# penghao-wu/vstar

Hardware: AMD Instinct MI355X
Metric: searched crops/sec (336x336 tiles, 7B VSM bf16) (higher is better)
Workload: dtype bf16; 1 GPU; BASELINE config 2: 32-crop batches/GPU, CLIP-ViT-L/14@336 (P=576) + LLaMA-7B prefill S=640 + OWL-ViT-B/16@768 + det/SAM heads, records all-gathered per step; seq_len=640, parallelism=dp1

## Files before the change

### include/vstar_hip.h

```cpp
#ifndef VSTAR_HIP_H
#define VSTAR_HIP_H

#include <stdint.h>
#include <stddef.h>

#ifdef __cplusplus
extern "C" {
#endif

#define VSTAR_ABI_VERSION 1

enum { VSTAR_F32 = 0, VSTAR_F16 = 1, VSTAR_BF16 = 2 };

enum {
  VSTAR_OK = 0,
  VSTAR_ERR_INVALID = -1,
  VSTAR_ERR_STATE = -2,
  VSTAR_ERR_MISSING = -3,
  VSTAR_ERR_HIP = -4,
  VSTAR_ERR_NOMEM = -5
};

typedef struct vstar_config {
  int32_t abi_version;
// ... 49 lines not shown
#define VSTAR_F_DEVICE_INPUTS  2u
#define VSTAR_F_DEVICE_OUTPUT  4u
#define VSTAR_F_NO_SYNC        8u
#define VSTAR_F_INTERNAL_PIXELS 16u
#define VSTAR_F_SHARE_PREFIX   32u
int vstar_vsm_score_batch(vstar_handle* h, int B, const uint16_t* clip_pix, const uint16_t* owl_pix,
                          const int32_t* ids, int L, const int32_t* loc_pos,
                          const int32_t* verify_pos, int n_verify, unsigned flags, vstar_result* out);

int vstar_vsm_score_grouped(vstar_handle* h, int G, int T, const uint16_t* clip_pix, const uint16_t* owl_pix,
                            const int32_t* prefix_ids, int Lp, const int32_t* suffix_ids, int Ls, const int32_t* loc_in_suffix,
                            const int32_t* verify_in_suffix, int n_verify, unsigned flags, vstar_result* out);

int vstar_image_set(vstar_handle* h, const uint8_t* rgb, int height, int width);
int vstar_preprocess_crops(vstar_handle* h, int B, const int32_t* boxes_xyxy);

#define VSTAR_MAX_IMAGE_SLOTS 64
int vstar_image_set_slot(vstar_handle* h, int slot, const uint8_t* rgb, int height, int width);
int vstar_preprocess_crops_slots(vstar_handle* h, int B, const int32_t* boxes_xyxy, const int32_t* slots);
int vstar_image_set_slot_async(vstar_handle* h, int slot, const uint8_t* rgb, int height, int width);

int vstar_vsm_generate(vstar_handle* h, const uint16_t* clip_pix_bf16, const int32_t* ids, int L, int max_new_tokens,
                       int eos_id, unsigned flags, int32_t* out_ids, int32_t* n_out);

int vstar_upsample_mask(vstar_handle* h, const float* lowres, int h_out, int w_out, float* out);
int vstar_upsample_mask_ex(vstar_handle* h, const float* lowres, int h_out, int w_out, int clamp_min0, float* out);

int vstar_heatmap_stats(vstar_handle* h, const float* lowres, int h_out, int w_out, int n_rects, const int32_t* rects_xywh,
                        double* out);
int vstar_heatmap_stats_batch(vstar_handle* h, int n, const float* lowres, const int32_t* out_hw, const int32_t* n_rects,
                              const int32_t* rects_xywh, double* out);

int64_t vstar_debug_read(vstar_handle* h, const char* name, float* out, int64_t cap);

void* vstar_stream(vstar_handle* h);

#define VSTAR_COMM_ID_BYTES 128
int vstar_comm_unique_id(uint8_t* id_out );
int vstar_comm_init(vstar_handle* h, const uint8_t* id, int world, int rank);
int vstar_allgather_results(vstar_handle* h, const vstar_result* local_dev, int n_local, vstar_result* gathered_dev, unsigned flags);
int vstar_comm_destroy(vstar_handle* h);

int vstar_profile_enable(vstar_handle* h, int on);
int vstar_profile_read(vstar_handle* h, double* gemm_ms, int64_t* gemm_launches, double* gemm_flops);
int vstar_profile_read_fp8(vstar_handle* h, double* gemm_ms, int64_t* gemm_launches, double* gemm_flops);

enum { VSTAR_EPI_NONE = 0, VSTAR_EPI_QUICK_GELU = 1, VSTAR_EPI_GELU = 2, VSTAR_EPI_RELU = 3, VSTAR_EPI_SILU_MUL = 4,
       VSTAR_EPI_NOSYNC = 0x100,
       VSTAR_EPI_TILE128 = 0x200,
       VSTAR_EPI_TILE256 = 0x400,
       VSTAR_EPI_TILE4W = 0x800    };

int vstar_op_gemm(void* stream, const uint16_t* dev_A, int64_t lda, const uint16_t* dev_W, const uint16_t* dev_bias,
                  const uint16_t* dev_residual, int64_t ldr, void* dev_C, int64_t ldc, int out_f32,
                  int M, int N, int K, int epilogue);
int vstar_op_gemm_norm(void* stream, const uint16_t* dev_A, int64_t lda, const uint16_t* dev_W, const uint16_t* dev_bias,
                       const uint16_t* dev_residual, int64_t ldr, void* dev_C, int64_t ldc, int M, int N, int K, int epilogue,
                       const float* dev_row_scale, float* dev_sumsq_out, int sumsq_ld);
int vstar_op_rms_rstd(void* stream, const uint16_t* dev_x, const float* dev_partials, int ld, int rows, int cols, float eps,
                      float* dev_r);
int vstar_op_ln_fold(void* stream, uint16_t* dev_W, uint16_t* dev_bias, const uint16_t* dev_g, const uint16_t* dev_b_ln,
                     int n_rows, int K);
int vstar_op_gemm_last_tile(void);
int vstar_op_gemm_plan(int M, int N, int K, int epilogue, int has_residual, int fused_rope, int cus);
int vstar_op_gemm_fp8(void* stream, const uint16_t* dev_A, const uint16_t* dev_W, const uint16_t* dev_bias,
                      const uint16_t* dev_residual, uint16_t* dev_C, int M, int N, int K, int epilogue, int iters, float* gemm_ms);
size_t vstar_op_mx_scale_bytes(int rows, int cols);
int64_t vstar_op_mx_scale_offset(int row, int k_block, int rows);
int vstar_op_quantize_mx(void* stream, const uint16_t* dev_X, uint8_t* dev_q, uint8_t* dev_scales, int rows, int cols);
int vstar_op_gemm_mx(void* stream, const uint8_t* dev_Aq, const uint8_t* dev_a_scales, const float* dev_row_scale, const uint16_t* dev_W,
                     const uint16_t* dev_residual, uint16_t* dev_C, uint8_t* dev_C8, uint8_t* dev_c_scales, float* dev_sumsq, int M, int N, int K,
                     int epilogue, int iters, float* gemm_ms);
int vstar_op_gemm_fp8_mxout(void* stream, const uint16_t* dev_A, const uint16_t* dev_W, uint8_t* dev_C8, uint8_t* dev_c_scales, int M, int N,
                            int K, int iters, float* gemm_ms);
int vstar_op_attention_mx(void* stream, const uint16_t* dev_qkv, uint8_t* dev_out8, uint8_t* dev_scales, int B, int S, int H);
int vstar_w8a8_mx_active(vstar_handle* h);
int vstar_op_layernorm(void* stream, const uint16_t* dev_x, const uint16_t* dev_gamma, const uint16_t* dev_beta,
                       uint16_t* dev_y, int rows, int cols, float eps);
int vstar_op_rmsnorm(void* stream, const uint16_t* dev_x, const uint16_t* dev_gamma, uint16_t* dev_y,
                     int rows, int cols, float eps);
int vstar_op_attention(void* stream, uint16_t* dev_qkv, uint16_t* dev_out, void* dev_workspace, size_t workspace_bytes,
                       int B, int S, int H, int D, int causal, float rope_theta);
size_t vstar_op_attention_workspace(int B, int S, int H, int D);

int vstar_op_owl_class_logits(void* stream, const float* dev_emb, int ld, int Q, const uint16_t* dev_query, float* dev_out,
                              int out_stride_crop, int B, int rows_per_crop, int img_div);
int vstar_op_owl_box_finish(void* stream, const float* dev_raw, int ld, float* dev_out, int out_stride_crop, int B, int grid, int img_div);
int vstar_op_upsample2x_im2col3x3(void* stream, const uint16_t* dev_src, uint16_t* dev_A, int B, int h, int w, int C);
int vstar_op_hyper_mask(void* stream, const uint16_t* dev_hyper, const uint16_t* dev_up, float* dev_out, int out_stride_crop, int B,
                        int npix, int C);
int vstar_op_im2col_patch(void* stream, const uint16_t* dev_pix, uint16_t* dev_A, int B, int I, int ps, int Kpad);
int vstar_op_vit_assemble_tokens(void* stream, const uint16_t* dev_patch, const uint16_t* dev_cls, const uint16_t* dev_pos,
                                 uint16_t* dev_tokens, int B, int P, int C);
int vstar_op_llm_embed_text(void* stream, const int32_t* dev_ids, int L, int img_col, int P, const uint16_t* dev_table, int vocab,
                            uint16_t* dev_x, int B, int C);
int vstar_op_add_bcast(void* stream, const uint16_t* dev_a, const uint16_t* dev_b, uint16_t* dev_out, int64_t rows, int cols,
                       int64_t b_rows);
int vstar_op_add_bcast_repeat(void* stream, const uint16_t* dev_a, const uint16_t* dev_b, uint16_t* dev_out, int n_out, int rep,
                              int rows_per, int cols);
int vstar_op_bcast_rows(void* stream, const uint16_t* dev_src, uint16_t* dev_dst, int nrep, int64_t rep_stride, int nrows, int cols,
                        int64_t ld);
int vstar_op_owl_cls_mul(void* stream, const uint16_t* dev_x, uint16_t* dev_y, int B, int N, int C);
int vstar_op_gather_rows(void* stream, const uint16_t* dev_x, const int32_t* dev_idx, uint16_t* dev_y, int rows, int cols);
int vstar_op_argmax_rows(void* stream, const float* dev_x, int rows, int cols, int ld, int32_t* dev_out, int out_stride);
int vstar_op_layernorm_ex(void* stream, const uint16_t* dev_x, const uint16_t* dev_gamma, const uint16_t* dev_beta, uint16_t* dev_y,
                          int rows, int cols, float eps, const int32_t* dev_row_index, int act);
int vstar_op_rmsnorm_ex(void* stream, const uint16_t* dev_x, const uint16_t* dev_gamma, uint16_t* dev_y, int rows, int cols, float eps,
                        const int32_t* dev_row_index);
int vstar_op_ln_rstd(void* stream, const uint16_t* dev_x, const float* dev_partials, int ld, int rows, int cols, float eps,
                     float* dev_r);
int vstar_op_scale_cols(void* stream, uint16_t* dev_W, const uint16_t* dev_w, int64_t rows, int K);
int vstar_op_fill(void* stream, uint16_t* dev_v, int64_t n, float value);
int vstar_op_quantize_rows_fp8(void* stream, const uint16_t* dev_x, int64_t ldx, uint8_t* dev_q, int64_t ldq, float* dev_scale, int rows,
                               int cols);
int vstar_op_rmsnorm_quant_fp8(void* stream, const uint16_t* dev_x, const uint16_t* dev_gamma, uint8_t* dev_q, float* dev_scale, int rows,
                               int cols, float eps);
int vstar_op_small_attention(void* stream, const uint16_t* dev_q, const uint16_t* dev_k, const uint16_t* dev_v, uint16_t* dev_out, int B,
                             int Nq, int Nk, int H, int D);

#ifdef __cplusplus
}
#endif
#endif
```

### vstar_amd/_lib.py

```python
from __future__ import annotations

import ctypes
import os
from ctypes import POINTER, c_char_p, c_double, c_float, c_int, c_int32, c_int64, c_size_t, c_uint, c_uint16, c_void_p

from .config import CVqaConfig, CVstarConfig, MASK_RES, MAX_VERIFY, N_BOXES

LIB_PATH = os.environ.get("VSTAR_LIB") or os.path.join(os.path.dirname(os.path.abspath(__file__)), "libvstar_hip.so")

EXPORTS = [
    "vstar_create", "vstar_destroy", "vstar_last_error", "vstar_load_tensor", "vstar_finalize_weights",
    "vstar_vsm_score_batch", "vstar_upsample_mask", "vstar_debug_read", "vstar_stream", "vstar_profile_enable",
    "vstar_profile_read", "vstar_profile_read_fp8", "vstar_op_gemm", "vstar_op_layernorm", "vstar_op_rmsnorm", "vstar_op_attention",
    "vstar_op_attention_workspace", "vstar_image_set", "vstar_preprocess_crops", "vstar_heatmap_stats", "vstar_heatmap_stats_batch", "vstar_vsm_generate", "vstar_op_gemm_fp8",
    "vstar_op_gemm_last_tile", "vstar_op_gemm_plan", "vstar_op_gemm_norm", "vstar_op_rms_rstd", "vstar_op_ln_fold", "vstar_upsample_mask_ex", "vstar_vsm_score_grouped",
    "vstar_image_set_slot", "vstar_image_set_slot_async", "vstar_preprocess_crops_slots", "vstar_comm_unique_id", "vstar_comm_init", "vstar_allgather_results",
    "vstar_comm_destroy", "vstar_build_source_hash", "vstar_op_mx_scale_bytes", "vstar_op_mx_scale_offset", "vstar_op_quantize_mx",
    "vstar_op_gemm_mx", "vstar_op_gemm_fp8_mxout", "vstar_op_attention_mx", "vstar_w8a8_mx_active",
    "vstar_op_owl_class_logits", "vstar_op_owl_box_finish", "vstar_op_upsample2x_im2col3x3", "vstar_op_hyper_mask",
    "vstar_op_im2col_patch", "vstar_op_vit_assemble_tokens", "vstar_op_llm_embed_text", "vstar_op_add_bcast",
    "vstar_op_add_bcast_repeat", "vstar_op_bcast_rows", "vstar_op_owl_cls_mul", "vstar_op_gather_rows", "vstar_op_argmax_rows",
    "vstar_op_layernorm_ex", "vstar_op_rmsnorm_ex", "vstar_op_ln_rstd", "vstar_op_scale_cols", "vstar_op_fill",
    "vstar_op_quantize_rows_fp8", "vstar_op_rmsnorm_quant_fp8", "vstar_op_small_attention",
]

EXPORTS_VQA = [
    "vstar_vqa_create", "vstar_vqa_destroy", "vstar_vqa_last_error", "vstar_vqa_load_tensor", "vstar_vqa_finalize_weights",
    "vstar_vqa_encode_images", "vstar_vqa_forward", "vstar_vqa_debug_read", "vstar_vqa_last_forward_ms", "vstar_vqa_op_gemm",
    "vstar_vqa_forward_sample", "vstar_vqa_op_sample", "vstar_vqa_forward_beam", "vstar_vqa_kv_reorder", "vstar_vqa_kv_copy",
    "vstar_vqa_op_beam_select", "vstar_vqa_forward_score", "vstar_vqa_op_score",
    "vstar_vqa_decode_weight_bits", "vstar_vqa_op_quantize_w8", "vstar_vqa_op_gemm_w8",
    "vstar_vqa_op_quantize_w4", "vstar_vqa_op_gemm_w4",
    "vstar_vqa_kv_cache_format", "vstar_vqa_kv_cache_bytes", "vstar_vqa_op_kv_quantize",
    "vstar_vqa_forward_verify", "vstar_vqa_op_verify",
    "vstar_vqa_forward_edits", "vstar_vqa_forward_sample_edits", "vstar_vqa_forward_verify_edits", "vstar_vqa_op_edit",
    "vstar_vqa_logit_edit_capacity",
]

F32, F16, BF16 = 0, 1, 2
MAX_IMAGE_SLOTS = 64
EPI_NONE, EPI_QUICK_GELU, EPI_GELU, EPI_RELU, EPI_SILU_MUL = range(5)
EPI_NOSYNC, EPI_TILE128, EPI_TILE256, EPI_TILE4W = 0x100, 0x200, 0x400, 0x800
TILE_4W = 2564
F_SKIP_OWL, F_DEVICE_INPUTS, F_DEVICE_OUTPUT, F_NO_SYNC, F_INTERNAL_PIXELS, F_SHARE_PREFIX = 1, 2, 4, 8, 16, 32


class VstarResult(ctypes.Structure):
    _fields_ = [
        ("pred_logits", c_float * N_BOXES),
        ("pred_boxes", c_float * (N_BOXES * 4)),
        ("lowres_mask", c_float * (MASK_RES * MASK_RES)),
        ("tf_argmax", c_int32 * MAX_VERIFY),
    ]


RESULT_FLOATS = ctypes.sizeof(VstarResult) // 4


class VqaSampling(ctypes.Structure):
    _fields_ = [
        ("temperature", c_float),
        ("top_k", c_int32),
        ("top_p", c_float),
        ("step", ctypes.c_uint32),
        ("seed", ctypes.c_uint64),
        ("stream", ctypes.c_uint64),
    ]


class VqaLogitEdits(ctypes.Structure):
    _fields_ = [
        ("off", c_void_p),
        ("tok", c_void_p),
        ("penalty", c_void_p),
    ]


class VstarError(RuntimeError):
    pass


_lib = None


def load() -> ctypes.CDLL:
    global _lib
    if _lib is not None:
        return _lib
    if not os.path.exists(LIB_PATH):
        raise VstarError(f"{LIB_PATH} not built — run __graft_entry__.build() (hipcc --offload-arch=gfx950); "
                         "there is no CPU fallback for the HIP engine")
    import torch
    lib = ctypes.CDLL(LIB_PATH)
    H = c_void_p
    lib.vstar_create.argtypes = [POINTER(CVstarConfig), c_int, POINTER(H)]
    lib.vstar_create.restype = c_int
    lib.vstar_destroy.argtypes = [H]
    lib.vstar_destroy.restype = None
    lib.vstar_last_error.argtypes = [H]
    lib.vstar_last_error.restype = c_char_p
    lib.vstar_build_source_hash.argtypes = []
# ... 6 lines not shown
                                          c_void_p]
    lib.vstar_vsm_score_batch.restype = c_int
    lib.vstar_vsm_score_grouped.argtypes = [H, c_int, c_int, c_void_p, c_void_p, c_void_p, c_int, c_void_p, c_int, c_void_p, c_void_p, c_int,
                                            c_uint, c_void_p]
    lib.vstar_vsm_score_grouped.restype = c_int
    lib.vstar_vsm_generate.argtypes = [H, c_void_p, c_void_p, c_int, c_int, c_int, c_uint, c_void_p, c_void_p]
    lib.vstar_vsm_generate.restype = c_int
    lib.vstar_image_set.argtypes = [H, c_void_p, c_int, c_int]
    lib.vstar_image_set.restype = c_int
    lib.vstar_preprocess_crops.argtypes = [H, c_int, c_void_p]
    lib.vstar_preprocess_crops.restype = c_int
    lib.vstar_image_set_slot.argtypes = [H, c_int, c_void_p, c_int, c_int]
    lib.vstar_image_set_slot.restype = c_int
    lib.vstar_image_set_slot_async.argtypes = [H, c_int, c_void_p, c_int, c_int]
    lib.vstar_image_set_slot_async.restype = c_int
    lib.vstar_preprocess_crops_slots.argtypes = [H, c_int, c_void_p, c_void_p]
    lib.vstar_preprocess_crops_slots.restype = c_int
    lib.vstar_comm_unique_id.argtypes = [c_void_p]
    lib.vstar_comm_unique_id.restype = c_int
    lib.vstar_comm_init.argtypes = [H, c_void_p, c_int, c_int]
    lib.vstar_comm_init.restype = c_int
    lib.vstar_allgather_results.argtypes = [H, c_void_p, c_int, c_void_p, ctypes.c_uint]
    lib.vstar_allgather_results.restype = c_int
    lib.vstar_comm_destroy.argtypes = [H]
    lib.vstar_comm_destroy.restype = c_int
    lib.vstar_heatmap_stats.argtypes = [H, c_void_p, c_int, c_int, c_int, c_void_p, c_void_p]
    lib.vstar_heatmap_stats.restype = c_int
    lib.vstar_heatmap_stats_batch.argtypes = [H, c_int, c_void_p, c_void_p, c_void_p, c_void_p, c_void_p]
    lib.vstar_heatmap_stats_batch.restype = c_int
    lib.vstar_upsample_mask.argtypes = [H, c_void_p, c_int, c_int, c_void_p]
    lib.vstar_upsample_mask.restype = c_int
    lib.vstar_upsample_mask_ex.argtypes = [H, c_void_p, c_int, c_int, c_int, c_void_p]
    lib.vstar_upsample_mask_ex.restype = c_int
    lib.vstar_debug_read.argtypes = [H, c_char_p, c_void_p, c_int64]
    lib.vstar_debug_read.restype = c_int64
    lib.vstar_stream.argtypes = [H]
    lib.vstar_stream.restype = c_void_p
    lib.vstar_profile_enable.argtypes = [H, c_int]
    lib.vstar_profile_enable.restype = c_int
    lib.vstar_profile_read.argtypes = [H, POINTER(c_double), POINTER(c_int64), POINTER(c_double)]
    lib.vstar_profile_read.restype = c_int
    lib.vstar_profile_read_fp8.argtypes = [H, POINTER(c_double), POINTER(c_int64), POINTER(c_double)]
    lib.vstar_profile_read_fp8.restype = c_int
    lib.vstar_op_gemm.argtypes = [c_void_p, c_void_p, c_int64, c_void_p, c_void_p, c_void_p, c_int64, c_void_p, c_int64,
                                  c_int, c_int, c_int, c_int, c_int]
    lib.vstar_op_gemm.restype = c_int
    lib.vstar_op_gemm_norm.argtypes = [c_void_p, c_void_p, c_int64, c_void_p, c_void_p, c_void_p, c_int64, c_void_p, c_int64, c_int, c_int, c_int,
                                       c_int, c_void_p, c_void_p, c_int]
    lib.vstar_op_gemm_norm.restype = c_int
    lib.vstar_op_rms_rstd.argtypes = [c_void_p, c_void_p, c_void_p, c_int, c_int, c_int, c_float, c_void_p]
    lib.vstar_op_rms_rstd.restype = c_int
    lib.vstar_op_ln_fold.argtypes = [c_void_p, c_void_p, c_void_p, c_void_p, c_void_p, c_int, c_int]
    lib.vstar_op_ln_fold.restype = c_int
    lib.vstar_op_gemm_last_tile.argtypes = []
    lib.vstar_op_gemm_last_tile.restype = c_int
    lib.vstar_op_gemm_plan.argtypes = [c_int] * 7
    lib.vstar_op_gemm_plan.restype = c_int
    lib.vstar_op_gemm_fp8.argtypes = [c_void_p, c_void_p, c_void_p, c_void_p, c_void_p, c_void_p, c_int, c_int, c_int, c_int, c_int,
                                      POINTER(c_float)]
    lib.vstar_op_gemm_fp8.restype = c_int
    lib.vstar_op_mx_scale_bytes.argtypes = [c_int, c_int]
    lib.vstar_op_mx_scale_bytes.restype = c_size_t
    lib.vstar_op_mx_scale_offset.argtypes = [c_int, c_int, c_int]
    lib.vstar_op_mx_scale_offset.restype = ctypes.c_int64
    lib.vstar_op_quantize_mx.argtypes = [c_void_p, c_void_p, c_void_p, c_void_p, c_int, c_int]
    lib.vstar_op_quantize_mx.restype = c_int
    lib.vstar_op_gemm_mx.argtypes = [c_void_p] * 10 + [c_int, c_int, c_int, c_int, c_int, POINTER(c_float)]
    lib.vstar_op_gemm_mx.restype = c_int
    lib.vstar_op_gemm_fp8_mxout.argtypes = [c_void_p, c_void_p, c_void_p, c_void_p, c_void_p, c_int, c_int, c_int, c_int, POINTER(c_float)]
    lib.vstar_op_gemm_fp8_mxout.restype = c_int
    lib.vstar_op_attention_mx.argtypes = [c_void_p, c_void_p, c_void_p, c_void_p, c_int, c_int, c_int]
    lib.vstar_op_attention_mx.restype = c_int
    lib.vstar_w8a8_mx_active.argtypes = [c_void_p]
    lib.vstar_w8a8_mx_active.restype = c_int
    lib.vstar_op_layernorm.argtypes = [c_void_p, c_void_p, c_void_p, c_void_p, c_void_p, c_int, c_int, c_float]
    lib.vstar_op_layernorm.restype = c_int
    lib.vstar_op_rmsnorm.argtypes = [c_void_p, c_void_p, c_void_p, c_void_p, c_int, c_int, c_float]
    lib.vstar_op_rmsnorm.restype = c_int
    lib.vstar_op_attention.argtypes = [c_void_p, c_void_p, c_void_p, c_void_p, c_size_t, c_int, c_int, c_int, c_int, c_int,
                                       c_float]
    lib.vstar_op_attention.restype = c_int
    lib.vstar_op_attention_workspace.argtypes = [c_int, c_int, c_int, c_int]
    lib.vstar_op_attention_workspace.restype = c_size_t
    V, I, L, F = c_void_p, c_int, c_int64, c_float
    for name, args in {
        "owl_class_logits": [V, I, I, V, V, I, I, I, I], "owl_box_finish": [V, I, V, I, I, I, I],
        "upsample2x_im2col3x3": [V, V, I, I, I, I], "hyper_mask": [V, V, V, I, I, I, I],
        "im2col_patch": [V, V, I, I, I, I], "vit_assemble_tokens": [V, V, V, V, I, I, I],
        "llm_embed_text": [V, I, I, I, V, I, V, I, I], "add_bcast": [V, V, V, L, I, L],
        "add_bcast_repeat": [V, V, V, I, I, I, I], "bcast_rows": [V, V, I, L, I, I, L], "owl_cls_mul": [V, V, I, I, I],
        "gather_rows": [V, V, V, I, I], "argmax_rows": [V, I, I, I, V, I],
        "layernorm_ex": [V, V, V, V, I, I, F, V, I], "rmsnorm_ex": [V, V, V, I, I, F, V], "ln_rstd": [V, V, I, I, I, F, V],
        "scale_cols": [V, V, L, I], "fill": [V, L, F], "quantize_rows_fp8": [V, L, V, L, V, I, I],
        "rmsnorm_quant_fp8": [V, V, V, V, I, I, F], "small_attention": [V, V, V, V, I, I, I, I, I],
    }.items():
        fn = getattr(lib, "vstar_op_" + name)
        fn.argtypes = [c_void_p] + args
        fn.restype = c_int
    lib.vstar_vqa_create.argtypes = [POINTER(CVqaConfig), c_int, POINTER(H)]
    lib.vstar_vqa_create.restype = c_int
    lib.vstar_vqa_destroy.argtypes = [H]
    lib.vstar_vqa_destroy.restype = None
    lib.vstar_vqa_last_error.argtypes = [H]
    lib.vstar_vqa_last_error.restype = c_char_p
    lib.vstar_vqa_load_tensor.argtypes = [H, c_char_p, c_void_p, c_int, c_int, POINTER(c_int64)]
    lib.vstar_vqa_load_tensor.restype = c_int
    lib.vstar_vqa_finalize_weights.argtypes = [H]
    lib.vstar_vqa_finalize_weights.restype = c_int
    lib.vstar_vqa_encode_images.argtypes = [H, c_int, c_void_p, c_int]
    lib.vstar_vqa_encode_images.restype = c_int
    lib.vstar_vqa_forward.argtypes = [H, c_int, c_void_p, c_void_p, c_void_p, c_void_p, c_void_p, c_int, c_void_p, c_void_p,
                                      c_void_p]
    lib.vstar_vqa_forward.restype = c_int
    lib.vstar_vqa_forward_sample.argtypes = [H, c_int, c_void_p, c_void_p, c_void_p, c_void_p, c_void_p, c_int, c_void_p,
                                             c_void_p, c_void_p]
    lib.vstar_vqa_forward_sample.restype = c_int
    lib.vstar_vqa_op_sample.argtypes = [c_void_p, c_int, c_int, c_int, c_int64, c_void_p, c_void_p, c_void_p, c_void_p]
    lib.vstar_vqa_op_sample.restype = c_int
    lib.vstar_vqa_forward_beam.argtypes = [H, c_int, c_void_p, c_void_p, c_void_p, c_void_p, c_void_p, c_int, c_void_p,
                                           c_void_p, c_int, c_void_p, c_int, c_void_p, c_void_p, c_void_p, c_void_p]
    lib.vstar_vqa_forward_beam.restype = c_int
    lib.vstar_vqa_kv_reorder.argtypes = [H, c_int, c_void_p, c_void_p, c_int, c_int]
    lib.vstar_vqa_kv_reorder.restype = c_int
    lib.vstar_vqa_kv_copy.argtypes = [H, c_int, c_int, c_int, c_int]
    lib.vstar_vqa_kv_copy.restype = c_int
    lib.vstar_vqa_op_beam_select.argtypes = [c_void_p, c_int, c_int, c_int, c_int64, c_void_p, c_int, c_void_p, c_int, c_void_p,
                                             c_void_p, c_void_p, c_void_p]
    lib.vstar_vqa_op_beam_select.restype = c_int
    lib.vstar_vqa_forward_score.argtypes = [H, c_int, c_void_p, c_void_p, c_void_p, c_void_p, c_void_p, c_int, c_void_p,
                                            c_void_p, c_void_p, c_void_p]
    lib.vstar_vqa_forward_score.restype = c_int
    lib.vstar_vqa_op_score.argtypes = [c_void_p, c_int, c_int, c_int, c_int64, c_void_p, c_void_p, c_void_p, c_void_p]
    lib.vstar_vqa_op_score.restype = c_int
    lib.vstar_vqa_forward_verify.argtypes = [H, c_int, c_void_p, c_void_p, c_void_p, c_void_p, c_void_p, c_int, c_void_p,
                                             c_void_p, c_void_p, c_int, c_void_p, c_void_p, c_void_p]
    lib.vstar_vqa_forward_verify.restype = c_int
    lib.vstar_vqa_op_verify.argtypes = [c_void_p, c_int, c_int, c_int, c_int64, c_void_p, c_int, c_void_p, c_void_p, c_void_p,
                                        c_void_p]
    lib.vstar_vqa_op_verify.restype = c_int
    lib.vstar_vqa_forward_edits.argtypes = lib.vstar_vqa_forward.argtypes + [c_void_p]
    lib.vstar_vqa_forward_edits.restype = c_int
    lib.vstar_vqa_forward_sample_edits.argtypes = lib.vstar_vqa_forward_sample.argtypes + [c_void_p]
    lib.vstar_vqa_forward_sample_edits.restype = c_int
    lib.vstar_vqa_forward_verify_edits.argtypes = lib.vstar_vqa_forward_verify.argtypes + [c_void_p]
    lib.vstar_vqa_forward_verify_edits.restype = c_int
    lib.vstar_vqa_op_edit.argtypes = [c_void_p, c_int, c_int, c_int, c_int64, c_void_p, c_void_p, c_void_p]
    lib.vstar_vqa_op_edit.restype = c_int
    lib.vstar_vqa_logit_edit_capacity.argtypes = [H]
    lib.vstar_vqa_logit_edit_capacity.restype = c_int64
    lib.vstar_vqa_op_gemm.argtypes = [c_void_p, c_void_p, c_void_p, c_void_p, c_void_p, c_int, c_int, c_int, c_int, c_int,
                                      c_void_p, c_float]
    lib.vstar_vqa_op_gemm.restype = c_int
    lib.vstar_vqa_decode_weight_bits.argtypes = [H]
    lib.vstar_vqa_decode_weight_bits.restype = c_int
    lib.vstar_vqa_op_quantize_w8.argtypes = [c_void_p, c_int, c_int, c_void_p, c_void_p, c_void_p]
    lib.vstar_vqa_op_quantize_w8.restype = c_int
    lib.vstar_vqa_op_gemm_w8.argtypes = [c_void_p, c_void_p, c_void_p, c_void_p, c_void_p, c_void_p, c_int, c_int, c_int, c_int, c_int,
                                         c_void_p, c_float, c_int]
    lib.vstar_vqa_op_gemm_w8.restype = c_int
    lib.vstar_vqa_kv_cache_format.argtypes = [H]
    lib.vstar_vqa_kv_cache_format.restype = c_int
    lib.vstar_vqa_kv_cache_bytes.argtypes = [H]
    lib.vstar_vqa_kv_cache_bytes.restype = ctypes.c_int64
    lib.vstar_vqa_op_kv_quantize.argtypes = [c_void_p, c_int, c_void_p, c_void_p, c_void_p]
    lib.vstar_vqa_op_kv_quantize.restype = c_int
    lib.vstar_vqa_op_quantize_w4.argtypes = [c_void_p, c_int, c_int, c_void_p, c_void_p, c_void_p]
# ... 23 lines not shown
```

### vstar_amd/csrc/attention.hip

```cpp
#include "common.hpp"
#include "kernels.hpp"
#include "mx.hpp"
#include <cstdlib>
#include <type_traits>

#ifndef ATTN_EARLY_V
#define ATTN_EARLY_V(D) ((D) == 128)
#endif

namespace VS_NS {

namespace {

__global__ void rope_kernel(lp_t* __restrict__ qkv, const lp_t* __restrict__ cos_sin, int rows, int S, int H, int D, int grp_R0,
                            int grp_Lc) {
  const int half = D >> 1;
  const int vec_per_head = half >> 3;
  const int per_row = 2 * H * vec_per_head;
  const int64_t idx = (int64_t)blockIdx.x * blockDim.x + threadIdx.x;
  if (idx >= (int64_t)rows * per_row) return;
  const int row = (int)(idx / per_row);
  int rem = (int)(idx - (int64_t)row * per_row);
  const int which = rem / (H * vec_per_head);
  rem -= which * H * vec_per_head;
  const int h = rem / vec_per_head;
  const int d0 = (rem - h * vec_per_head) * 8;
  int pos = row % S;
  if (grp_R0 > 0 && pos >= grp_R0) pos = grp_Lc + ((pos - grp_R0) & 31);
  lp_t* base = qkv + (int64_t)row * (3 * H * D) + which * (H * D) + h * D;
  const lpx8 x1 = *(const lpx8*)(base + d0);
  const lpx8 x2 = *(const lpx8*)(base + d0 + half);
  const lpx8 c = *(const lpx8*)(cos_sin + (int64_t)pos * D + d0);
  const lpx8 sn = *(const lpx8*)(cos_sin + (int64_t)pos * D + half + d0);
  lpx8 o1, o2;
#pragma unroll
  for (int e = 0; e < 8; ++e) {
    const float a = lp2f((lp_t)x1[e]), b = lp2f((lp_t)x2[e]);
    const float cs = lp2f((lp_t)c[e]), si = lp2f((lp_t)sn[e]);
    o1[e] = (short)f2lp(rlp(a * cs) + rlp(-b * si));
    o2[e] = (short)f2lp(rlp(b * cs) + rlp(a * si));
  }
  *(lpx8*)(base + d0) = o1;
  *(lpx8*)(base + d0 + half) = o2;
}

template <int D, bool CAUSAL, bool MXO = false>
__global__ __launch_bounds__(256) void attn2_kernel(const lp_t* __restrict__ qkv, lp_t* __restrict__ out, int S, int H,
                                                    float scale_log2e, int grp_R0, int grp_Lc, int nqb, uint8_t* __restrict__ mxs = nullptr,
                                                    int m128 = 0) {
  constexpr int KS = D / 16, DB = D / 32;
  constexpr int KT = 64;
  constexpr int NBUF = 128 / KT;
  constexpr int KBYTES = KT * D * 2;
  constexpr int KCH = D / 8;
  constexpr int KROWS_PER_INST = 64 / KCH;
  constexpr int K_INST = KT / KROWS_PER_INST / 4;
  static_assert(K_INST >= 1, "tile too small for 4 DMA waves");
  extern __shared__ __attribute__((aligned(16))) char smem[];
  typedef const __attribute__((address_space(1))) void* gptr_t;
  typedef __attribute__((address_space(3))) void* lptr_t;
  const int lane = threadIdx.x & 63;
  const int wave = __builtin_amdgcn_readfirstlane(threadIdx.x >> 6);
  int h, b, qblk;
  {
    const int total = (int)gridDim.x, L = (int)blockIdx.x;
    const int per = total >> 3, rem = total & 7, x = L & 7;
    const int v = (x < rem ? x * (per + 1) : rem * (per + 1) + (x - rem) * per) + (L >> 3);
    qblk = v % nqb;
    const int hb = v / nqb;
    h = hb % H;
    b = hb / H;
  }
  const int q0b = (CAUSAL ? nqb - 1 - qblk : qblk) * 128;
  const int q0 = q0b + wave * 32;
  const bool active = q0 < S;
  const int qi = lane & 31, h2 = lane >> 5;
  const int query = q0 + qi;
  const int qrow = query < S ? query : S - 1;
  const int64_t ld = 3 * (int64_t)H * D;
  const lp_t* Kg = qkv + (int64_t)b * S * ld + (int64_t)H * D + h * D;
  const lp_t* Vg = qkv + (int64_t)b * S * ld + 2 * (int64_t)H * D + h * D;

  const bool sfx = CAUSAL && grp_R0 > 0 && q0b >= grp_R0;
  const int nsh = sfx ? (grp_Lc + KT - 1) / KT : 0;
  auto key0 = [&](int t) { return sfx ? (t < nsh ? t * KT : q0b + (t - nsh) * KT) : t * KT; };

#ifndef ATTN_BUFFER_DMA
#define ATTN_BUFFER_DMA 1
#endif
  const int64_t ldb = ld * (int64_t)sizeof(lp_t);
  uint32_t koffs[K_INST], voffs[K_INST];
  const lp_t* ksrc[K_INST];
  int krow_l[K_INST];
#pragma unroll
  for (int i = 0; i < K_INST; ++i) {
    const int row = (i * 4 + wave) * KROWS_PER_INST + lane / KCH;
    const int ch = lane % KCH;
    const int sw = (D == 64) ? ((row >> 1) & 7) : (row & 15);
    krow_l[i] = row;
    ksrc[i] = Kg + (ch ^ sw) * 8;
    koffs[i] = (uint32_t)(row * ldb + (ch ^ sw) * 16);
  }
  const lp_t* vsrc[K_INST];
#pragma unroll
  for (int i = 0; i < K_INST; ++i) {
    const int row = (i * 4 + wave) * KROWS_PER_INST + lane / KCH;
    const int ch = lane % KCH;
    const int gq = (D == 64) ? ((row >> 1) & 1) : (row & 3);
    vsrc[i] = Vg + (ch ^ (gq << 2)) * 8;
    voffs[i] = (uint32_t)(row * ldb + (ch ^ (gq << 2)) * 16);
  }
  const uint32_t span = (uint32_t)((int64_t)(S - 1) * ldb + D * (int)sizeof(lp_t));
#if defined(__HIP_DEVICE_COMPILE__)
  const __amdgpu_buffer_rsrc_t krsrc = __builtin_amdgcn_make_buffer_rsrc((void*)Kg, 0, (int)span, 0x00020000);
  const __amdgpu_buffer_rsrc_t vrsrc = __builtin_amdgcn_make_buffer_rsrc((void*)Vg, 0, (int)span, 0x00020000);
#endif
  auto stage = [&](int t) {
    char* base = smem + (t % NBUF) * 2 * KBYTES;
    const int kt0 = key0(t);
#if defined(__HIP_DEVICE_COMPILE__)
    if constexpr (ATTN_BUFFER_DMA) {
      const int soff = __builtin_amdgcn_readfirstlane((int)(kt0 * ldb));
#pragma unroll
      for (int i = 0; i < K_INST; ++i)
        __builtin_amdgcn_raw_ptr_buffer_load_lds(krsrc, (lptr_t)(base + (i * 4 + wave) * 1024), 16, koffs[i], soff, 0, 0);
#pragma unroll
      for (int i = 0; i < K_INST; ++i)
        __builtin_amdgcn_raw_ptr_buffer_load_lds(vrsrc, (lptr_t)(base + KBYTES + (i * 4 + wave) * 1024), 16, voffs[i], soff, 0, 0);
      return;
// ... 62 lines not shown
      const lpx8 kf = *(const lpx8*)(smem + koff[ks] + SBASE);
      sacc = mfma_32x32x16(kf, qf[ks], sacc);
    }
    s4_t vlo[2][DB], vhi[2][DB];
#define ATTN_V_READS()                                                                                                         \
  _Pragma("unroll") for (int j = 0; j < 2; ++j) _Pragma("unroll") for (int db = 0; db < DB; ++db) {                              \
    asm volatile("ds_read_b64_tr_b16 %0, %1 offset:%2" : "=v"(vlo[j][db]) : "v"(voff[db]), "i"(SBASE + 16 * j * (D * 2)));       \
    asm volatile("ds_read_b64_tr_b16 %0, %1 offset:%2" : "=v"(vhi[j][db]) : "v"(voff[db]), "i"(SBASE + (16 * j + 8) * (D * 2))); \
  }
    constexpr bool EARLY_V = ATTN_EARLY_V(D);
    if constexpr (EARLY_V) { ATTN_V_READS() }
    const bool causal_here = CAUSAL && !shared_tile;
    const bool need_mask = (kt0 + 32 > klimit) || (causal_here && kt0 + 31 > q0);
    if (need_mask) {
#pragma unroll
      for (int r = 0; r < 16; ++r) {
        const int key = kt0 + (r & 3) + 8 * (r >> 2) + 4 * h2;
        const bool masked = (key >= klimit) || (causal_here && key > query);
        sacc[r] = masked ? -1e30f : sacc[r];
      }
    }
    constexpr float BIG = 65536.0f;
    float p[16];
    float rs = 0.f;
#pragma unroll
    for (int r = 0; r < 16; ++r) {
      p[r] = __builtin_amdgcn_exp2f(sacc[r]);
      rs += p[r];
    }
    if (first || __any(!(rs <= BIG))) {
      float mx = sacc[0];
#pragma unroll
      for (int r = 1; r < 16; ++r) mx = fmaxf(mx, sacc[r]);
      mx = fmaxf(mx, __shfl_xor(mx, 32, 64));
      const float delta = first ? fmaxf(mx, -1e4f) : fmaxf(mx, 0.f);
      const float alpha = first ? 1.0f : __builtin_amdgcn_exp2f(-delta);
      l *= alpha;
#pragma unroll
      for (int db = 0; db < DB; ++db)
#pragma unroll
        for (int r = 0; r < 16; ++r) oacc[db][r] *= alpha;
      m += delta;
#pragma unroll
      for (int r = 0; r < 16; ++r) negm[r] = -m;
      rs = 0.f;
#pragma unroll
      for (int r = 0; r < 16; ++r) {
        p[r] = __builtin_amdgcn_exp2f(sacc[r] - delta);
        rs += p[r];
      }
      first = false;
    }
    l += rs;
    if constexpr (!EARLY_V) { ATTN_V_READS() }
#undef ATTN_V_READS
#pragma unroll
    for (int j = 0; j < 2; ++j)
#pragma unroll
      for (int db = 0; db < DB; ++db) asm volatile("s_waitcnt lgkmcnt(0)" : "+v"(vlo[j][db]), "+v"(vhi[j][db]));
#pragma unroll
    for (int j = 0; j < 2; ++j) {
      lpx8 pb;
#pragma unroll
      for (int i = 0; i < 8; ++i) pb[i] = (short)f2lp(p[8 * j + i]);
#pragma unroll
      for (int db = 0; db < DB; ++db) {
        const lpx8 vf = (lpx8){vlo[j][db][0], vlo[j][db][1], vlo[j][db][2], vlo[j][db][3],
                               vhi[j][db][0], vhi[j][db][1], vhi[j][db][2], vhi[j][db][3]};
        oacc[db] = mfma_32x32x16(vf, pb, oacc[db]);
      }
    }
  };

  auto tile = [&](auto SLOT_, int t) {
    __builtin_amdgcn_sched_barrier(0);
    asm volatile("s_waitcnt vmcnt(0) lgkmcnt(0)\n\ts_barrier" ::: "memory");
    __builtin_amdgcn_sched_barrier(0);
    if (t + 1 < nkt) stage(t + 1);
    if (active) {
      subtile(SLOT_, std::integral_constant<int, 0>{}, t);
      subtile(SLOT_, std::integral_constant<int, 1>{}, t);
    }
  };
  stage(0);
  for (int t = 0; t < nkt; t += 2) {
    tile(std::integral_constant<int, 0>{}, t);
    if (t + 1 < nkt) tile(std::integral_constant<int, 1>{}, t + 1);
  }
  l += __shfl_xor(l, 32, 64);

  if constexpr (MXO) {
    const float inv = 1.0f / l;
    const int row = b * S + query;
    uint8_t* op8 = (uint8_t*)out + (int64_t)row * ((int64_t)H * D) + h * D + 16 * h2;
#pragma unroll
    for (int db = 0; db < DB; ++db) {
      float f[16], mx = 0.f;
#pragma unroll
      for (int r = 0; r < 16; ++r) {
        f[r] = rlp(oacc[db][r] * inv);
        mx = fmaxf(mx, fabsf(f[r]));
      }
      mx = mx_max_halves(mx);
      const uint32_t e8 = mx_e8m0(mx);
      const float is = mx_inv_scale(e8);
      uint32_t pk[4];
#pragma unroll
      for (int g = 0; g < 4; ++g) pk[g] = mx_pack4(f[g * 4] * is, f[g * 4 + 1] * is, f[g * 4 + 2] * is, f[g * 4 + 3] * is);
      const auto s02 = __builtin_amdgcn_permlane32_swap(pk[0], pk[2], false, false);
      const auto s13 = __builtin_amdgcn_permlane32_swap(pk[1], pk[3], false, false);
      if (active && query < S) {
        typedef __attribute__((ext_vector_type(4))) unsigned int u32x4;
        const u32x4 o = {s02[0], s02[1], s13[0], s13[1]};
        *(u32x4*)(op8 + db * 32) = o;
        if (h2 == 0) mxs[mx_scale_offset(row, h * DB + db, m128)] = (uint8_t)e8;
      }
    }
    return;
  }
#ifndef ATTN_WIDE_STORES
#define ATTN_WIDE_STORES 1
#endif
  if constexpr (ATTN_WIDE_STORES) {
    const float inv = 1.0f / l;
    lp_t* op = out + ((int64_t)b * S + query) * ((int64_t)H * D) + h * D + 16 * h2;
    const bool wr = active && query < S;
#pragma unroll
    for (int db = 0; db < DB; ++db) {
      uint32_t pk[4][2];
#pragma unroll
      for (int g = 0; g < 4; ++g)
#pragma unroll
        for (int k = 0; k < 2; ++k)
          pk[g][k] = (uint32_t)(uint16_t)f2lp(oacc[db][g * 4 + 2 * k] * inv) | ((uint32_t)(uint16_t)f2lp(oacc[db][g * 4 + 2 * k + 1] * inv) << 16);
      typedef __attribute__((ext_vector_type(4))) unsigned int u32x4;
#pragma unroll
      for (int gp = 0; gp < 2; ++gp) {
        const auto s0 = __builtin_amdgcn_permlane32_swap(pk[gp][0], pk[gp + 2][0], false, false);
        const auto s1 = __builtin_amdgcn_permlane32_swap(pk[gp][1], pk[gp + 2][1], false, false);
        const u32x4 o = {s0[0], s1[0], s0[1], s1[1]};
        if (wr) *(u32x4*)(op + db * 32 + gp * 8) = o;
      }
    }
    return;
  }
  if (active && query < S) {
    const float inv = 1.0f / l;
    lp_t* op = out + ((int64_t)b * S + query) * ((int64_t)H * D) + h * D + 4 * h2;
#pragma unroll
    for (int db = 0; db < DB; ++db)
#pragma unroll
      for (int g = 0; g < 4; ++g) {
        lpx4 o;
#pragma unroll
        for (int e = 0; e < 4; ++e) o[e] = (short)f2lp(oacc[db][g * 4 + e] * inv);
        *(lpx4*)(op + db * 32 + g * 8) = o;
      }
  }
}

template <int D>
__global__ __launch_bounds__(256) void small_attn_kernel(const lp_t* __restrict__ q, const lp_t* __restrict__ k,
                                                         const lp_t* __restrict__ v, lp_t* __restrict__ out, int B,
                                                         int Nq, int Nk, int H, float scale) {
  const int lane = threadIdx.x & 63;
  const int64_t wid = (int64_t)blockIdx.x * 4 + (threadIdx.x >> 6);
  if (wid >= (int64_t)B * H * Nq) return;
  const int qi = (int)(wid % Nq);
  const int h = (int)((wid / Nq) % H);
  const int b = (int)(wid / ((int64_t)Nq * H));
// ... 58 lines not shown
__global__ __launch_bounds__(256) void small_attn_fewkeys_kernel(const lp_t* __restrict__ q, const lp_t* __restrict__ k,
                                                                 const lp_t* __restrict__ v, lp_t* __restrict__ out,
                                                                 int B, int Nq, int Nk, int H, float scale) {
  const int64_t idx = (int64_t)blockIdx.x * blockDim.x + threadIdx.x;
  if (idx >= (int64_t)B * H * Nq) return;
  const int h = (int)(idx % H);
  const int qi = (int)((idx / H) % Nq);
  const int b = (int)(idx / ((int64_t)H * Nq));
  const int C = H * D;
  const lp_t* qp = q + ((int64_t)b * Nq + qi) * C + h * D;
  float qv[D];
#pragma unroll
  for (int d0 = 0; d0 < D; d0 += 8) {
    const lpx8 t = *(const lpx8*)(qp + d0);
#pragma unroll
    for (int e = 0; e < 8; ++e) qv[d0 + e] = lp2f((lp_t)t[e]);
  }
  float sc[MAXK];
  float mx = -1e30f;
#pragma unroll
  for (int j = 0; j < MAXK; ++j) {
    sc[j] = -1e30f;
    if (j < Nk) {
      const lp_t* kp = k + ((int64_t)b * Nk + j) * C + h * D;
      float a = 0.f;
#pragma unroll
      for (int d0 = 0; d0 < D; d0 += 8) {
        const lpx8 t = *(const lpx8*)(kp + d0);
#pragma unroll
        for (int e = 0; e < 8; ++e) a += qv[d0 + e] * lp2f((lp_t)t[e]);
      }
      sc[j] = rlp(rlp(a) * scale);
      mx = fmaxf(mx, sc[j]);
    }
  }
  float sum = 0.f;
#pragma unroll
  for (int j = 0; j < MAXK; ++j) {
    sc[j] = j < Nk ? __expf(sc[j] - mx) : 0.f;
    sum += sc[j];
  }
  const float inv = 1.0f / sum;
  float o[D];
#pragma unroll
  for (int d = 0; d < D; ++d) o[d] = 0.f;
#pragma unroll
  for (int j = 0; j < MAXK; ++j) {
    if (j < Nk) {
      const float pr = rlp(sc[j] * inv);
      const lp_t* vp = v + ((int64_t)b * Nk + j) * C + h * D;
#pragma unroll
      for (int d0 = 0; d0 < D; d0 += 8) {
        const lpx8 t = *(const lpx8*)(vp + d0);
#pragma unroll
        for (int e = 0; e < 8; ++e) o[d0 + e] += pr * lp2f((lp_t)t[e]);
      }
    }
  }
  lp_t* op = out + ((int64_t)b * Nq + qi) * C + h * D;
#pragma unroll
  for (int d0 = 0; d0 < D; d0 += 8) {
    lpx8 t;
#pragma unroll
    for (int e = 0; e < 8; ++e) t[e] = (short)f2lp(o[d0 + e]);
    *(lpx8*)(op + d0) = t;
  }
}

}

hipError_t attn_prepare(lp_t* qkv, const lp_t* cos_sin, int B, int S, int H, int D, hipStream_t s, int grp_R0, int grp_Lc) {
  if (D != 64 && D != 128) return hipErrorInvalidValue;
  if (cos_sin) {
    const int64_t n = (int64_t)B * S * 2 * H * (D / 16);
    hipLaunchKernelGGL(rope_kernel, dim3((unsigned)((n + 255) / 256)), dim3(256), 0, s, qkv, cos_sin, B * S, S, H, D, grp_R0, grp_Lc);
  }
  return hipGetLastError();
}

template <int D, bool CAUSAL, bool MXO = false>
static hipError_t launch_attn2(const lp_t* qkv, lp_t* out, int B, int S, int H, float sl, hipStream_t s, int grp_R0 = 0,
                               int grp_Lc = 0, uint8_t* mxs = nullptr) {
  constexpr int LDS = 4 * 64 * D * 2;
  static bool attr_done = false;
  auto kern = attn2_kernel<D, CAUSAL, MXO>;
  if (!attr_done) {
    hipError_t e = hipFuncSetAttribute((const void*)kern, hipFuncAttributeMaxDynamicSharedMemorySize, LDS);
    if (e != hipSuccess) return e;
    attr_done = true;
  }
  const int nqb = (S + 127) / 128;
  dim3 grid((unsigned)(nqb * H * B));
  hipLaunchKernelGGL(kern, grid, dim3(256), LDS, s, qkv, out, S, H, sl, grp_R0, grp_Lc, nqb, mxs, (B * S) >> 7);
  return hipGetLastError();
}

hipError_t attn_forward(const lp_t* qkv, lp_t* out, int B, int S, int H, int D, int causal, float scale, hipStream_t s, int grp_R0,
                        int grp_Lc) {
  if (D != 64 && D != 128) return hipErrorInvalidValue;
  if (grp_R0 > 0 && (!causal || D != 128 || grp_R0 % 128 || grp_Lc <= 0 || grp_Lc > grp_R0 || (S - grp_R0) % 32)) return hipErrorInvalidValue;
  const float sl = scale * 1.4426950408889634f;
  if (D == 64) return causal ? launch_attn2<64, true>(qkv, out, B, S, H, sl, s) : launch_attn2<64, false>(qkv, out, B, S, H, sl, s);
  return causal ? launch_attn2<128, true>(qkv, out, B, S, H, sl, s, grp_R0, grp_Lc) : launch_attn2<128, false>(qkv, out, B, S, H, sl, s);
}

hipError_t attn_forward_mx(const lp_t* qkv, uint8_t* out8, uint8_t* scales, int B, int S, int H, float scale, hipStream_t s, int grp_R0,
                           int grp_Lc) {
#ifdef VSTAR_LP_F16
  return hipErrorInvalidValue;
#else
  if ((int64_t)B * S % 128 || !out8 || !scales) return hipErrorInvalidValue;
  if (grp_R0 > 0 && (grp_R0 % 128 || grp_Lc <= 0 || grp_Lc > grp_R0 || (S - grp_R0) % 32)) return hipErrorInvalidValue;
  return launch_attn2<128, true, true>(qkv, (lp_t*)out8, B, S, H, scale * 1.4426950408889634f, s, grp_R0, grp_Lc, scales);
#endif
}

hipError_t small_attention(const lp_t* q, const lp_t* k, const lp_t* v, lp_t* out, int B, int Nq, int Nk, int H,
                           int D, hipStream_t s) {
  if (Nk > 40 * 64) return hipErrorInvalidValue;
  const int64_t waves = (int64_t)B * H * Nq;
  dim3 grid((unsigned)((waves + 3) / 4));
  const float scale = 1.0f / sqrtf((float)D);
  if (Nk <= 8 && (D == 16 || D == 32)) {
    const int64_t threads = (int64_t)B * H * Nq;
    dim3 g((unsigned)((threads + 255) / 256));
    if (D == 16) hipLaunchKernelGGL((small_attn_fewkeys_kernel<16, 8>), g, dim3(256), 0, s, q, k, v, out, B, Nq, Nk, H, scale);
    else hipLaunchKernelGGL((small_attn_fewkeys_kernel<32, 8>), g, dim3(256), 0, s, q, k, v, out, B, Nq, Nk, H, scale);
    return hipGetLastError();
  }
  if (D == 32) hipLaunchKernelGGL(small_attn_kernel<32>, grid, dim3(256), 0, s, q, k, v, out, B, Nq, Nk, H, scale);
  else if (D == 16) hipLaunchKernelGGL(small_attn_kernel<16>, grid, dim3(256), 0, s, q, k, v, out, B, Nq, Nk, H, scale);
  else return hipErrorInvalidValue;
  return hipGetLastError();
}

}
```

Baseline: 144.2 crops/s.

## Add software-pipelined skewed softmax/PV schedule to attention kernel

Adds a SKEW variant of the flash attention kernel that defers each subtile's P·V MFMAs into the next subtile. The next tile's exp2/softmax and transposed V LDS reads are interleaved with the previous tile's MFMAs. It also uses a lazy rescaling scheme: the running max is only recentred when the row sum exceeds a threshold, which removes the per-tile max/rescale work. The variant is selected at runtime by an env var or debug API and is on by default. It adds register pressure and complexity, and the lazy rescaling carries a small numerical risk.

```diff
diff --git a/include/vstar_hip.h b/include/vstar_hip.h
--- a/include/vstar_hip.h
+++ b/include/vstar_hip.h
@@ -155,6 +155,7 @@
 int vstar_op_attention(void* stream, uint16_t* dev_qkv, uint16_t* dev_out, void* dev_workspace, size_t workspace_bytes,
                        int B, int S, int H, int D, int causal, float rope_theta);
 size_t vstar_op_attention_workspace(int B, int S, int H, int D);
+int vstar_debug_attention_schedule(int schedule);
 
 int vstar_op_owl_class_logits(void* stream, const float* dev_emb, int ld, int Q, const uint16_t* dev_query, float* dev_out,
                               int out_stride_crop, int B, int rows_per_crop, int img_div);
diff --git a/vstar_amd/_lib.py b/vstar_amd/_lib.py
--- a/vstar_amd/_lib.py
+++ b/vstar_amd/_lib.py
@@ -16,7 +16,7 @@
     "vstar_op_gemm_last_tile", "vstar_op_gemm_plan", "vstar_op_gemm_norm", "vstar_op_rms_rstd", "vstar_op_ln_fold", "vstar_upsample_mask_ex", "vstar_vsm_score_grouped",
     "vstar_image_set_slot", "vstar_image_set_slot_async", "vstar_preprocess_crops_slots", "vstar_comm_unique_id", "vstar_comm_init", "vstar_allgather_results",
     "vstar_comm_destroy", "vstar_build_source_hash", "vstar_op_mx_scale_bytes", "vstar_op_mx_scale_offset", "vstar_op_quantize_mx",
-    "vstar_op_gemm_mx", "vstar_op_gemm_fp8_mxout", "vstar_op_attention_mx", "vstar_w8a8_mx_active",
+    "vstar_op_gemm_mx", "vstar_op_gemm_fp8_mxout", "vstar_op_attention_mx", "vstar_w8a8_mx_active", "vstar_debug_attention_schedule",
     "vstar_op_owl_class_logits", "vstar_op_owl_box_finish", "vstar_op_upsample2x_im2col3x3", "vstar_op_hyper_mask",
     "vstar_op_im2col_patch", "vstar_op_vit_assemble_tokens", "vstar_op_llm_embed_text", "vstar_op_add_bcast",
     "vstar_op_add_bcast_repeat", "vstar_op_bcast_rows", "vstar_op_owl_cls_mul", "vstar_op_gather_rows", "vstar_op_argmax_rows",
@@ -189,6 +189,8 @@
     lib.vstar_op_attention.restype = c_int
     lib.vstar_op_attention_workspace.argtypes = [c_int, c_int, c_int, c_int]
     lib.vstar_op_attention_workspace.restype = c_size_t
+    lib.vstar_debug_attention_schedule.argtypes = [c_int]
+    lib.vstar_debug_attention_schedule.restype = c_int
     V, I, L, F = c_void_p, c_int, c_int64, c_float
     for name, args in {
         "owl_class_logits": [V, I, I, V, V, I, I, I, I], "owl_box_finish": [V, I, V, I, I, I, I],
diff --git a/vstar_amd/csrc/attention.hip b/vstar_amd/csrc/attention.hip
--- a/vstar_amd/csrc/attention.hip
+++ b/vstar_amd/csrc/attention.hip
@@ -6,6 +6,22 @@
 
 #ifndef ATTN_EARLY_V
 #define ATTN_EARLY_V(D) ((D) == 128)
+#endif
+
+#ifndef ATTN_SCHED_DEFAULT
+#define ATTN_SCHED_DEFAULT 1
+#endif
+#ifndef VSTAR_LP_F16
+extern "C" {
+int vstar_attention_schedule_state = [] { const char* e = getenv("VSTAR_ATTN_SCHED"); return e ? (atoi(e) != 0) : ATTN_SCHED_DEFAULT; }();
+int vstar_debug_attention_schedule(int schedule) {
+  const int prev = vstar_attention_schedule_state;
+  if (schedule == 0 || schedule == 1) vstar_attention_schedule_state = schedule;
+  return prev;
+}
+}
+#else
+extern "C" int vstar_attention_schedule_state;
 #endif
 
 namespace VS_NS {
@@ -44,7 +60,7 @@
   *(lpx8*)(base + d0 + half) = o2;
 }
 
-template <int D, bool CAUSAL, bool MXO = false>
+template <int D, bool CAUSAL, bool MXO = false, bool SKEW = false>
 __global__ __launch_bounds__(256) void attn2_kernel(const lp_t* __restrict__ qkv, lp_t* __restrict__ out, int S, int H,
                                                     float scale_log2e, int grp_R0, int grp_Lc, int nqb, uint8_t* __restrict__ mxs = nullptr,
                                                     int m128 = 0) {
@@ -273,10 +289,166 @@
       subtile(SLOT_, std::integral_constant<int, 1>{}, t);
     }
   };
-  stage(0);
-  for (int t = 0; t < nkt; t += 2) {
-    tile(std::integral_constant<int, 0>{}, t);
-    if (t + 1 < nkt) tile(std::integral_constant<int, 1>{}, t + 1);
+  if constexpr (!SKEW) {
+    stage(0);
+    for (int t = 0; t < nkt; t += 2) {
+      tile(std::integral_constant<int, 0>{}, t);
+      if (t + 1 < nkt) tile(std::integral_constant<int, 1>{}, t + 1);
+    }
+  }
+
+  if constexpr (SKEW) {
+    s4_t pvlo[2][DB], pvhi[2][DB];
+    lpx8 ppb[2];
+    auto subtile_skew = [&](auto SLOT_, auto ST_, auto FIRST_, int t) __attribute__((always_inline)) {
+      constexpr int SLOT = decltype(SLOT_)::value, st = decltype(ST_)::value;
+      constexpr bool FIRST = decltype(FIRST_)::value;
+      constexpr int SBASE = SLOT * 2 * KBYTES + st * 32 * (D * 2);
+      const int kt0 = key0(t) + st * 32;
+      const bool shared_tile = sfx && t < nsh;
+      const int klimit = shared_tile ? grp_Lc : S;
+      if constexpr (!FIRST) {
+        if (kt0 >= (shared_tile ? grp_Lc : kend)) return;
+        if (sfx && !shared_tile && kt0 != q0) return;
+        if (CAUSAL && !shared_tile && kt0 > q0 + 31) return;
+      }
+#ifndef ATTN_SKEW_KA
+#define ATTN_SKEW_KA(D) ((D) == 64 ? 1 : 4)
+#endif
+      constexpr int KA = ATTN_SKEW_KA(D);
+      lpx8 kf[KS];
+#pragma unroll
+      for (int ks = 0; ks < KA; ++ks) kf[ks] = *(const lpx8*)(smem + koff[ks] + SBASE);
+      __builtin_amdgcn_sched_barrier(0);
+      f32x16 sacc = negm;
+#pragma unroll
+      for (int ks = 0; ks < KS; ++ks) {
+        sacc = mfma_32x32x16(kf[ks], qf[ks], sacc);
+        if (ks + KA < KS) {
+          kf[ks + KA] = *(const lpx8*)(smem + koff[ks + KA] + SBASE);
+          __builtin_amdgcn_sched_barrier(0);
+        }
+      }
+      const bool causal_here = CAUSAL && !shared_tile;
+      const bool need_mask = (kt0 + 32 > klimit) || (causal_here && kt0 + 31 > q0);
+      if (need_mask) {
+#pragma unroll
+        for (int r = 0; r < 16; ++r) {
+          const int key = kt0 + (r & 3) + 8 * (r >> 2) + 4 * h2;
+          const bool masked = (key >= klimit) || (causal_here && key > query);
+          sacc[r] = masked ? -1e30f : sacc[r];
+        }
+      }
+      constexpr float BIG = 65536.0f;
+      float p[16];
+      float rs = 0.f;
+      lpx8 pbn[2];
+      auto recentre = [&]() __attribute__((always_inline)) {
+        float mx = sacc[0];
+#pragma unroll
+        for (int r = 1; r < 16; ++r) mx = fmaxf(mx, sacc[r]);
+        mx = fmaxf(mx, __shfl_xor(mx, 32, 64));
+        const float delta = FIRST ? fmaxf(mx, -1e4f) : fmaxf(mx, 0.f);
+        const float alpha = FIRST ? 1.0f : __builtin_amdgcn_exp2f(-delta);
+        l *= alpha;
+#pragma unroll
+        for (int db = 0; db < DB; ++db)
+#pragma unroll
+          for (int r = 0; r < 16; ++r) oacc[db][r] *= alpha;
+        m += delta;
+#pragma unroll
+        for (int r = 0; r < 16; ++r) negm[r] = -m;
+        rs = 0.f;
+#pragma unroll
+        for (int r = 0; r < 16; ++r) {
+          p[r] = __builtin_amdgcn_exp2f(sacc[r] - delta);
+          rs += p[r];
+        }
+#pragma unroll
+        for (int i = 0; i < 16; ++i) pbn[i >> 3][i & 7] = (short)f2lp(p[i]);
+      };
+#define ATTN_SKEW_VREAD(f)                                                                                                        \
+  {                                                                                                                               \
+    const int vo = voff[(f) % DB];                                                                                                \
+    asm volatile("ds_read_b64_tr_b16 %0, %1 offset:%2" : "=v"(pvlo[(f) / DB][(f) % DB]) : "v"(vo), "i"(SBASE + 16 * ((f) / DB) * (D * 2)));       \
+    asm volatile("ds_read_b64_tr_b16 %0, %1 offset:%2" : "=v"(pvhi[(f) / DB][(f) % DB]) : "v"(vo), "i"(SBASE + (16 * ((f) / DB) + 8) * (D * 2))); \
+  }
+      constexpr int NPV = 2 * DB;
+      if constexpr (FIRST) {
+#pragma unroll
+        for (int f = 0; f < NPV; ++f) ATTN_SKEW_VREAD(f)
+        recentre();
+      } else {
+#pragma unroll
+        for (int j = 0; j < 2; ++j)
+#pragma unroll
+          for (int db = 0; db < DB; ++db) asm volatile("s_waitcnt lgkmcnt(0)" : "+v"(pvlo[j][db]), "+v"(pvhi[j][db]));
+        uint32_t pw[8];
+        typedef __attribute__((ext_vector_type(2))) short s2_t;
+        typedef __attribute__((ext_vector_type(4))) unsigned int pw4_t;
+#define ATTN_SKEW_SOFTMAX(r)                                                                          \
+  {                                                                                                   \
+    p[r] = __builtin_amdgcn_exp2f(sacc[r]);                                                           \
+    rs += p[r];                                                                                       \
+    if ((r) & 1) {                                                                                    \
+      pw[(r) >> 1] = __builtin_bit_cast(uint32_t, (s2_t){(short)f2lp(p[(r) - 1]), (short)f2lp(p[r])}); \
+      asm volatile("" : "+v"(pw[(r) >> 1]));                                                          \
+    }                                                                                                 \
+  }
+#pragma unroll
+        for (int g = 0; g < NPV; ++g) {
+          const int j = g / DB, db = g % DB;
+          const lpx8 vf = (lpx8){pvlo[j][db][0], pvlo[j][db][1], pvlo[j][db][2], pvlo[j][db][3],
+                                 pvhi[j][db][0], pvhi[j][db][1], pvhi[j][db][2], pvhi[j][db][3]};
+          oacc[db] = mfma_32x32x16(vf, ppb[j], oacc[db]);
+          __builtin_amdgcn_sched_barrier(0);
+          ATTN_SKEW_SOFTMAX(g)
+          if (g > 0) ATTN_SKEW_VREAD(g - 1)
+          __builtin_amdgcn_sched_barrier(0);
+        }
+        ATTN_SKEW_VREAD(NPV - 1)
+#pragma unroll
+        for (int r = NPV; r < 16; ++r) ATTN_SKEW_SOFTMAX(r)
+#undef ATTN_SKEW_SOFTMAX
+        pbn[0] = __builtin_bit_cast(lpx8, (pw4_t){pw[0], pw[1], pw[2], pw[3]});
+        pbn[1] = __builtin_bit_cast(lpx8, (pw4_t){pw[4], pw[5], pw[6], pw[7]});
+        if (__any(!(rs <= BIG))) recentre();
+      }
+#undef ATTN_SKEW_VREAD
+      l += rs;
+      ppb[0] = pbn[0];
+      ppb[1] = pbn[1];
+    };
+    auto tile_skew = [&](auto SLOT_, auto FIRST_, int t) __attribute__((always_inline)) {
+      __builtin_amdgcn_sched_barrier(0);
+      asm volatile("s_waitcnt vmcnt(0) lgkmcnt(0)\n\ts_barrier" ::: "memory");
+      __builtin_amdgcn_sched_barrier(0);
+      if (t + 1 < nkt) stage(t + 1);
+      if (active) {
+        subtile_skew(SLOT_, std::integral_constant<int, 0>{}, FIRST_, t);
+        subtile_skew(SLOT_, std::integral_constant<int, 1>{}, std::false_type{}, t);
+      }
+    };
+    stage(0);
+    tile_skew(std::integral_constant<int, 0>{}, std::true_type{}, 0);
+    for (int t = 1; t < nkt; t += 2) {
+      tile_skew(std::integral_constant<int, 1>{}, std::false_type{}, t);
+      if (t + 1 < nkt) tile_skew(std::integral_constant<int, 0>{}, std::false_type{}, t + 1);
+    }
+    if (active) {
+#pragma unroll
+      for (int j = 0; j < 2; ++j)
+#pragma unroll
+        for (int db = 0; db < DB; ++db) asm volatile("s_waitcnt lgkmcnt(0)" : "+v"(pvlo[j][db]), "+v"(pvhi[j][db]));
+#pragma unroll
+      for (int j = 0; j < 2; ++j)
+#pragma unroll
+        for (int db = 0; db < DB; ++db) {
+          const lpx8 vf = (lpx8){pvlo[j][db][0], pvlo[j][db][1], pvlo[j][db][2], pvlo[j][db][3],
+                                 pvhi[j][db][0], pvhi[j][db][1], pvhi[j][db][2], pvhi[j][db][3]};
+          oacc[db] = mfma_32x32x16(vf, ppb[j], oacc[db]);
+        }
+    }
   }
   l += __shfl_xor(l, 32, 64);
 
@@ -501,12 +673,13 @@
 static hipError_t launch_attn2(const lp_t* qkv, lp_t* out, int B, int S, int H, float sl, hipStream_t s, int grp_R0 = 0,
                                int grp_Lc = 0, uint8_t* mxs = nullptr) {
   constexpr int LDS = 4 * 64 * D * 2;
-  static bool attr_done = false;
-  auto kern = attn2_kernel<D, CAUSAL, MXO>;
-  if (!attr_done) {
+  static bool attr_done[2] = {false, false};
+  const int skew = vstar_attention_schedule_state != 0;
+  auto kern = skew ? attn2_kernel<D, CAUSAL, MXO, true> : attn2_kernel<D, CAUSAL, MXO, false>;
+  if (!attr_done[skew]) {
     hipError_t e = hipFuncSetAttribute((const void*)kern, hipFuncAttributeMaxDynamicSharedMemorySize, LDS);
     if (e != hipSuccess) return e;
-    attr_done = true;
+    attr_done[skew] = true;
   }
   const int nqb = (S + 127) / 128;
   dim3 grid((unsigned)(nqb * H * B));
```

Result: no change. 144.3 crops/s, median of 2 (+0.0%).
